# vocdoni/gnark-crypto-primitives

Measured on AMD Instinct MI355X. Metric: proofs/sec, Arbo-160 Poseidon SMT-verifier circuit, Groth16/BN254, higher is better.
Workload: dtype u32x8 Montgomery (254-bit integer)

## Files before the change

gnark_crypto_primitives_amd/csrc/api.hip:

```cpp
#include <algorithm>

#include "zkmi_internal.h"
#include "comb_plan.h"
#include "ff29.h"
#include "ec29.h"

using namespace zk;

namespace zk {

int ensure_scratch(zkmi_ctx* ctx, DevBuf& s, size_t bytes, void** out) {
  if (s.bytes < bytes) {
    if (s.p) {
      hipStreamSynchronize(ctx->stream);
      if (ctx->stream2) hipStreamSynchronize(ctx->stream2);
      if (ctx->stream3) hipStreamSynchronize(ctx->stream3);
      hipFree(s.p);
      s.p = nullptr;
      s.bytes = 0;
    }
    hipError_t e = hipMalloc(&s.p, bytes);
    if (e != hipSuccess) {
      ctx->err = "hipMalloc(" + std::to_string(bytes) + " B) failed: " + hipGetErrorString(e) +
                 " (the working set of this batch does not fit beside the MSM tables: load the key"
                 " with zkmi_pk_desc.max_batch >= the batch size, or with a table_budget_bytes cap)";
      s.p = nullptr;
      return ZKMI_ERR_OOM;
    }
    s.bytes = bytes;
  }
  if (out) *out = s.p;
  return ZKMI_OK;
}

int require_idle(zkmi_ctx* ctx) {
  if (!ctx->sets[0].pending && !ctx->sets[1].pending) return ZKMI_OK;
  ctx->err = "a submitted prove batch is in flight; collect it first";
  return ZKMI_ERR_ARG;
}

template <class P>
__global__ __launch_bounds__(256) void field_mul_kernel(const Fp<P>* a, const Fp<P>* b, Fp<P>* r,
                                                        size_t n) {
  size_t i = (size_t)blockIdx.x * blockDim.x + threadIdx.x;
  const size_t stride = (size_t)gridDim.x * blockDim.x;
  for (; i < n; i += stride) r[i] = mul(a[i], b[i]);
}

template <class P>
// ... 207 lines not shown
  const size_t Bp = round_up(batch, 64);
  const SetBytes sb = prove_set_bytes(value_rows, (size_t)1 << pk->log_n, n_staged, batch, Bp);
  int rc;
  for (zkmi_ctx::ProveSet* T : {&ctx->sets[ctx->next_submit ^ 1], &S}) {
    if (T->pending) continue;
    if ((rc = ensure_scratch(ctx, T->slots, sb.slots)) || (rc = ensure_scratch(ctx, T->a, sb.abc)) ||
        (rc = ensure_scratch(ctx, T->b, sb.abc)) || (rc = ensure_scratch(ctx, T->c, sb.abc)) ||
        (rc = ensure_scratch(ctx, T->misc, sb.misc)) ||
        (rc = ensure_scratch(ctx, T->sums, sums_bytes(Bp))))
      return rc;
  }
  char* const staged = (char*)S.misc.p + Bp * 100;
  S.rs = S.misc.p;
  S.st = (char*)S.misc.p + Bp * 96;
  if (stage) *stage = staged;
  S.heavy_enqueued = false;
  S.batch = batch;
  S.Bp = Bp;
  S.pk = pk;
  *main = ctx->stream;
  ctx->stream = ctx->stream2;
  hipEventRecord(S.ev0, ctx->stream);
  const void* rs_dev;
  rc = device_view(ctx, rs, batch * 64, staged + batch * n_staged * 32, &rs_dev);
  if (!rc) rc = transpose_in(ctx, rs_dev, S.rs, 2, batch, Bp, 32);
  return rc ? prove_set_end(ctx, *main, rc) : ZKMI_OK;
}

int prove_set_end(zkmi_ctx* ctx, hipStream_t main, int rc) {
  zkmi_ctx::ProveSet& S = ctx->sets[ctx->next_submit];
  hipEventRecord(S.ev1, ctx->stream);
  ctx->stream = main;
  if (rc) {
    hipStreamSynchronize(ctx->stream2);
    return rc;
  }
  S.pending = true;
  ctx->next_submit ^= 1;
  return ZKMI_OK;
}

}

extern "C" {

int zkmi_init(int device, zkmi_ctx** out) {
  if (!out) return ZKMI_ERR_ARG;
  *out = nullptr;
  int count = 0;
  if (hipGetDeviceCount(&count) != hipSuccess || count <= 0) return ZKMI_ERR_NO_DEVICE;
  if (device < 0 || device >= count) return ZKMI_ERR_ARG;
  if (hipSetDevice(device) != hipSuccess) return ZKMI_ERR_HIP;
  auto* ctx = new zkmi_ctx();
  ctx->device = device;
  if (hipStreamCreateWithFlags(&ctx->stream, hipStreamNonBlocking) != hipSuccess) {
    delete ctx;
    return ZKMI_ERR_HIP;
  }
  if (hipStreamCreateWithFlags(&ctx->stream2, hipStreamNonBlocking) != hipSuccess) {
    hipStreamDestroy(ctx->stream);
    delete ctx;
    return ZKMI_ERR_HIP;
  }
  if (hipStreamCreateWithFlags(&ctx->stream3, hipStreamNonBlocking) != hipSuccess) {
    hipStreamDestroy(ctx->stream2);
    hipStreamDestroy(ctx->stream);
    delete ctx;
    return ZKMI_ERR_HIP;
  }
  for (auto& st : ctx->sets) {
    hipEventCreate(&st.ev0);
    hipEventCreate(&st.ev1);
    for (auto& e : st.evq) hipEventCreate(&e);
    for (auto& e : st.eva) hipEventCreate(&e);
    for (auto& p : st.msm_ev) {
      hipEventCreate(&p[0]);
      hipEventCreate(&p[1]);
    }
  }
  for (auto& e : ctx->ev) hipEventCreate(&e);
  for (auto& e : ctx->part_ev) hipEventCreateWithFlags(&e, hipEventDisableTiming);
  for (auto& e : ctx->acc_ev) hipEventCreateWithFlags(&e, hipEventDisableTiming);
  ctx->plans.reserve(32);
  *out = ctx;
  return ZKMI_OK;
}

void zkmi_destroy(zkmi_ctx* ctx) {
  if (!ctx) return;
  hipSetDevice(ctx->device);
  hipStreamSynchronize(ctx->stream);
  hipStreamSynchronize(ctx->stream2);
  hipStreamSynchronize(ctx->stream3);
  for (auto& st : ctx->sets) {
    if (st.ev0) hipEventDestroy(st.ev0);
    if (st.ev1) hipEventDestroy(st.ev1);
    for (auto& e : st.evq)
      if (e) hipEventDestroy(e);
    for (auto& e : st.eva)
      if (e) hipEventDestroy(e);
    for (auto& p : st.msm_ev) {
      if (p[0]) hipEventDestroy(p[0]);
      if (p[1]) hipEventDestroy(p[1]);
    }
  }
  hipStreamDestroy(ctx->stream2);
  hipStreamDestroy(ctx->stream3);
  for (auto& p : ctx->plans) free_plan(p);
  for (auto& st : ctx->sets)
    for (DevBuf* b : {&st.slots, &st.a, &st.b, &st.c, &st.misc, &st.sums, &st.commit})
      if (b->p) hipFree(b->p);
  for (DevBuf* b : {&ctx->ntt_tmp, &ctx->build_tmp, &ctx->msm_digits, &ctx->msm_sint,
                    &ctx->msm_rowvar, &ctx->msm_part[0], &ctx->msm_part[1], &ctx->side_part2, &ctx->side_part3})
    if (b->p) hipFree(b->p);
  witness_ring_free(ctx);
  for (auto& e : ctx->ev)
    if (e) hipEventDestroy(e);
  for (auto& e : ctx->part_ev)
    if (e) hipEventDestroy(e);
  for (auto& e : ctx->acc_ev)
    if (e) hipEventDestroy(e);
  hipStreamDestroy(ctx->stream);
  delete ctx;
}

const char* zkmi_last_error(zkmi_ctx* ctx) { return ctx ? ctx->err.c_str() : "null context"; }

int zkmi_sync(zkmi_ctx* ctx) {
  ZK_HIP(hipStreamSynchronize(ctx->stream));
  return ZKMI_OK;
}

void* zkmi_stream(zkmi_ctx* ctx) { return (void*)ctx->stream; }

int zkmi_field_mul(zkmi_ctx* ctx, int which, const void* a, const void* b, void* r, size_t n) {
  ZK_HIP(hipSetDevice(ctx->device));
  Staged sa(ctx), sb(ctx), sr(ctx);
  int rc;
  if ((rc = sa.in(a, n * 32)) || (rc = sb.in(b, n * 32)) || (rc = sr.out(r, n * 32))) return rc;
  if (n == 0) return ZKMI_OK;
  unsigned g = (unsigned)((n + 255) / 256);
  if (g > 8192) g = 8192;
  if (which == 0)
    hipLaunchKernelGGL((field_mul_kernel<FrParams>), dim3(g), dim3(256), 0, ctx->stream,
                       (const Fr*)sa.dev, (const Fr*)sb.dev, (Fr*)sr.dev, n);
  else
    hipLaunchKernelGGL((field_mul_kernel<FqParams>), dim3(g), dim3(256), 0, ctx->stream,
                       (const Fq*)sa.dev, (const Fq*)sb.dev, (Fq*)sr.dev, n);
  ZK_HIP(hipGetLastError());
  if ((rc = sr.finish())) return rc;
  ZK_HIP(hipStreamSynchronize(ctx->stream));
  return ZKMI_OK;
}
// ... 137 lines not shown
    if (rc != ZKMI_ERR_OOM || !may_relax) return rc;
    if (plan.comb) {
      if (plan.comb <= 8) return rc;
      plan = plan_comb(plan.comb - 1, plan.comb_signed != 0);
    } else if (plan.shared) {
      if (plan.bits[0] <= 4) return rc;
      plan = plan_shared(plan.bits[0] - 1);
    } else {
      if (plan.W >= 64) return rc;
      plan = plan_with_windows(plan.W + 1);
    }
  }
}

static bool window_bits_ok(int wb) {
  return wb == 0 || (wb >= 2 && wb <= 16) || (wb >= 104 && wb <= 116) ||
         (wb >= 202 && wb <= 220) || (wb >= 303 && wb <= 321);
}
static WinPlan plan_explicit(int wb) {
  return wb >= 300   ? plan_comb(wb - 300, true)
         : wb >= 200 ? plan_comb(wb - 200, false)
         : wb >= 100 ? plan_shared(wb - 100)
                     : plan_uniform(wb);
}
static double prove_working_set_bytes(uint32_t log_n, size_t n_slots, size_t n_in, size_t max_batch,
                                      size_t n_msm_max, size_t n_commitments) {
  const size_t Bp = round_up(max_batch ? max_batch : 1024, 64);
  const size_t n = (size_t)1 << log_n;
  const SetBytes sb = prove_set_bytes(n_slots, n, n_in, Bp, Bp);
  const double set = (double)(sb.slots + 3 * sb.abc + sb.misc + sums_bytes(Bp) +
                              commit_buffer_bytes(n_commitments, Bp));
  const double digits = 254.0 * (double)((n_msm_max + 15) / 16) * Bp * 4;
  const double sint = (double)n_msm_max * Bp * 32;
  const double partials = 2 * 21.0 * 254 * Bp * 256;
  const double ring = 3.0 * std::max(68e6, (double)n_in * 32 * 64);
  return 2 * set + (double)n * Bp * 32 + digits + sint + partials + ring + 2e9 + 1e9;
}
static double free_hbm_bytes() {
  size_t free_b = 0, total_b = 0;
  if (hipMemGetInfo(&free_b, &total_b) != hipSuccess) free_b = (size_t)64 << 30;
  return (double)free_b;
}
static double usable_table_bytes_standalone(size_t n) {
  const double ws = (double)n * 1024 * 32 * 2 + 254.0 * ((n + 15) / 16) * 1024 * 4 +
                    21.0 * 254 * 1024 * 256 + 3e9;
  const double usable = free_hbm_bytes() - ws;
  return usable > 0 ? usable : 0.0;
}

int zkmi_msm_bases_load(zkmi_ctx* ctx, int group, const void* bases, size_t n, int window_bits,
                        zkmi_msm_bases** out) {
  return zkmi_msm_bases_load_image(ctx, group, bases, n, window_bits, 0, out);
}

int zkmi_msm_bases_load_image(zkmi_ctx* ctx, int group, const void* bases, size_t n,
                              int window_bits, int image, zkmi_msm_bases** out) {
  ZK_HIP(hipSetDevice(ctx->device));
  if (!out) return ZKMI_ERR_ARG;
  if (image != 0 && image != 1) {
    ctx->err = "image must be 0 (x * 2^256) or 1 (x * 2^261)";
    return ZKMI_ERR_ARG;
  }
  if (!window_bits_ok(window_bits)) {
    ctx->err = "window_bits must be 0 (auto), in [2,16], 100 + [4,16], 200 + [2,20] or 300 + [3,21]";
    return ZKMI_ERR_ARG;
  }
  Staged sb(ctx);
// ... 596 lines not shown
    }
    if (!rc) rc = solve_rows(ctx, cs, slots, a, b, c, st, Bp, begin, cs->n_rows);
    if (!rc) rc = commit_finish_submit(ctx, S);
  }
  return prove_set_end(ctx, main, rc);
}

static int enqueue_heavy(zkmi_ctx* ctx, int si) {
  zkmi_ctx::ProveSet& S = ctx->sets[si];
  const zkmi_pk* pk = S.pk;
  const bool fd = S.f_domain;
  const size_t Bp = S.Bp, batch = S.batch, n = (size_t)1 << pk->log_n;
  NttPlan* plan;
  int rc = get_plan(ctx, (int)pk->log_n, &plan);
  if (rc) return rc;
  void* t0;
  if ((rc = ensure_scratch(ctx, ctx->ntt_tmp, n * Bp * 32, &t0))) return rc;
  SumsView v(S.sums.p, Bp);
  Fr* rs_bi = (Fr*)S.rs;
  Fr* slots = (Fr*)S.slots.p;
  ZK_HIP(hipStreamWaitEvent(ctx->stream, S.ev1, 0));
  hipEventRecord(S.evq[0], ctx->stream);
  Fr* h;
  if ((rc = pk->folded ? compute_ab_coset_bi(ctx, plan, (Fr*)S.a.p, (Fr*)S.b.p, (Fr*)t0, Bp,
                                             S.n_constraints, &h, fd)
                       : compute_h_bi(ctx, plan, (Fr*)S.a.p, (Fr*)S.b.p, (Fr*)S.c.p, (Fr*)t0, Bp,
                                      S.n_constraints, &h, fd)))
    return rc;
  hipEventRecord(S.evq[1], ctx->stream);
  S.msm_ev_used = 0;
  ctx->msm_ev_set = si;
  const bool d1 = pk->Z->plan.shared || pk->Z->plan.comb;
  const bool d2 = pk->B2->plan.shared || pk->B2->plan.comb;
  hipStream_t q3 = ctx->stream3;
  uint8_t* rv = nullptr;
  if (pk->A->plan.comb || pk->B2->plan.comb) {
    void* p;
    if ((rc = ensure_scratch(ctx, ctx->msm_rowvar, pk->n_wires, &p)) ||
        (rc = msm_rows_vary(ctx, slots, pk->n_wires, Bp, batch, (uint8_t*)p))) {
      ctx->msm_ev_set = -1;
      return rc;
    }
    rv = (uint8_t*)p;
  }
  if ((rc = msm_run(ctx, pk->A, slots, pk->a_wire, Bp, batch, v.sA, fd, d1 ? v.w1[0] : nullptr, q3,
                    rv)) ||
      (rc = msm_run(ctx, pk->B1, slots, pk->b_wire, Bp, batch, v.sB1, fd, d1 ? v.w1[1] : nullptr, q3,
                    rv)) ||
      (rc = msm_run(ctx, pk->K, slots, pk->k_wire, Bp, batch, v.sK, fd, d1 ? v.w1[2] : nullptr, q3,
                    rv)) ||
      (rc = msm_run(ctx, pk->Z, h, nullptr, Bp, batch, v.sZ, false, d1 ? v.w1[3] : nullptr, q3,
                    nullptr, true))) {
    ctx->msm_ev_set = -1;
    return rc;
  }
  hipEventRecord(S.evq[2], ctx->stream);
  rc = msm_run(ctx, pk->B2, slots, pk->b_wire, Bp, batch, v.sB2, fd, d2 ? v.w2 : nullptr, q3, rv);
  ctx->msm_ev_set = -1;
  if (rc) return rc;
  hipEventRecord(S.evq[3], ctx->stream);
  {
    hipStream_t main_stream = ctx->stream;
    ZK_HIP(hipStreamWaitEvent(q3, S.ev1, 0));
    ctx->stream = q3;
    hipLaunchKernelGGL(rs_prep_kernel, dim3((unsigned)(Bp / 64)), dim3(64), 0, q3, rs_bi, Bp);
    (void)((rc = msm_run(ctx, pk->D1, rs_bi, pk->idx3 + 0, Bp, batch, v.tR)) ||
           (rc = msm_run(ctx, pk->D1, rs_bi, pk->idx3 + 1, Bp, batch, v.tS)) ||
           (rc = msm_run(ctx, pk->D1, rs_bi, pk->idx3 + 2, Bp, batch, v.tNRS)) ||
           (rc = msm_run(ctx, pk->D2, rs_bi, pk->idx3 + 1, Bp, batch, v.tS2)));
    ctx->stream = main_stream;
    if (rc) return rc;
  }
  if ((rc = commit_pok(ctx, S))) return rc;
  hipEventRecord(S.evq[4], ctx->stream);
  S.heavy_enqueued = true;
  return ZKMI_OK;
}

int zkmi_prove_collect(zkmi_ctx* ctx, void* proofs_out, int32_t* status_out) {
  return zkmi_prove_collect_ex(ctx, proofs_out, status_out, nullptr);
}

int zkmi_prove_collect_ex(zkmi_ctx* ctx, void* proofs_out, int32_t* status_out,
                          void* commitments_out) {
  ZK_HIP(hipSetDevice(ctx->device));
  const int si = ctx->next_collect;
  zkmi_ctx::ProveSet& S = ctx->sets[si];
  if (!S.pending) {
    ctx->err = "prove: nothing submitted";
    return ZKMI_ERR_ARG;
  }
  if (!S.pk->commits.empty() && !commitments_out) {
    ctx->err = "prove: this key has commitments: collect with zkmi_prove_collect_ex";
    return ZKMI_ERR_ARG;
  }
  const zkmi_pk* pk = S.pk;
  const size_t batch = S.batch, Bp = S.Bp;
  int rc;
  if (!S.heavy_enqueued && (rc = enqueue_heavy(ctx, si))) return rc;
  SumsView v(S.sums.p, Bp);
  hipStream_t q3 = ctx->stream3;
  ZK_HIP(hipStreamWaitEvent(q3, S.evq[4], 0));
  hipEventRecord(S.eva[0], q3);
  if (pk->Z->plan.shared || pk->Z->plan.comb) {
    void* ws[4] = {v.w1[0], v.w1[1], v.w1[2], v.w1[3]};
    void* os[4] = {v.sA, v.sB1, v.sK, v.sZ};
    const zkmi_msm_bases* ms[4] = {pk->A, pk->B1, pk->K, pk->Z};
    bool same = true;
    for (int i = 0; i < 3; i++)
      same = same && (ms[i]->plan.comb != 0) == (pk->Z->plan.comb != 0) &&
             ms[i]->plan.comb_signed == pk->Z->plan.comb_signed &&
             (pk->Z->plan.comb || (ms[i]->plan.shared && ms[i]->plan.bits[0] == pk->Z->plan.bits[0]));
    if (same) {
      if ((rc = msm_horner_run(ctx, q3, 4, ms, ws, os, Bp))) return rc;
    } else {
      for (int i = 0; i < 4; i++)
        if ((rc = msm_horner_run(ctx, q3, 1, ms + i, ws + i, os + i, Bp))) return rc;
    }
  }
  if (pk->B2->plan.shared || pk->B2->plan.comb) {
    void* ws[1] = {v.w2};
    void* os[1] = {v.sB2};
    const zkmi_msm_bases* ms[1] = {pk->B2};
    if ((rc = msm_horner_run(ctx, q3, 1, ms, ws, os, Bp))) return rc;
  }
  PkConsts pc{pk->alpha, pk->beta1, pk->beta2};
  hipLaunchKernelGGL(assemble_kernel, dim3((unsigned)(Bp / 64)), dim3(64), 0, q3, v.sA, v.sB1, v.sK,
                     v.sZ, v.tR, v.tS, v.tNRS, (const Fr*)S.rs, Bp, pc, v.proofs);
  hipLaunchKernelGGL(assemble_g2_kernel, dim3((unsigned)(Bp / 64)), dim3(64), 0, q3, v.sB2, v.tS2,
                     Bp, pk->beta2, v.proofs);
  ZK_HIP(hipGetLastError());
  ZK_HIP(hipMemcpyAsync(proofs_out, v.proofs, batch * 256, hipMemcpyDefault, q3));
  ZK_HIP(hipMemcpyAsync(status_out, S.st, batch * 4, hipMemcpyDefault, q3));
  if (const size_t nc = pk->commits.size()) {
    const size_t pitch = (nc + 1) * 64;
// ... 47 lines not shown
```

gnark_crypto_primitives_amd/csrc/msm_impl.h:

```cpp
#pragma once
#include "zkmi_internal.h"
#include "ec29.h"
#include "comb_sign.h"

namespace zk {

ZK_HD Fq to_r261_domain(const Fq& x) {
  Fq k;
#pragma unroll
  for (int i = 0; i < 8; i++) k.v[i] = Fq29Params::k261(i);
  return mul(x, k);
}
ZK_HD Fq2 to_r261_domain(const Fq2& x) { return Fq2{to_r261_domain(x.c0), to_r261_domain(x.c1)}; }

template <class F>
struct SegInv {
  F *szz, *szzz, *spre;
  size_t T;
  F pref = F::one();
  __device__ SegInv(F* scratch, uint32_t t, uint32_t T_, uint32_t seg_len)
      : szz(scratch + t), szzz(scratch + (size_t)seg_len * T_ + t),
        spre(scratch + (size_t)2 * seg_len * T_ + t), T(T_) {}
  __device__ void push(Affine<F>* seg, uint32_t d, const F& x, const F& y, const F& zz,
                       const F& zzz) {
    seg[d].x = x;
    seg[d].y = y;
    szz[d * T] = zz;
    szzz[d * T] = zzz;
    spre[d * T] = pref;
    pref = mul(pref, zzz);
  }
  __device__ void finish(Affine<F>* seg, uint32_t len) {
    F inv = inverse(pref);
    for (uint32_t d = len; d-- > 0;) {
      const F zzz = szzz[d * T];
      const F izzz = mul(inv, spre[d * T]);
// ... 827 lines not shown
  size_t chunks = want;
  if (chunks < 1) chunks = 1;
  if (chunks > items) chunks = items;
  const uint32_t per_chunk = (uint32_t)((items + chunks - 1) / chunks);
  chunks = (items + per_chunk - 1) / per_chunk;
  uint32_t group = 1;
  while ((size_t)group * group < chunks) group++;
  return {chunks, per_chunk, group, (uint32_t)((chunks + group - 1) / group)};
}

template <class F>
static void reduce_partials(hipStream_t stream, const XYZZ<F>* partial, XYZZ<F>* mid, XYZZ<F>* out,
                            size_t Bp, const ChunkSplit& cs, int W, const XYZZ<F>* addend,
                            const uint32_t* counts) {
  const Part29<F>* in = (const Part29<F>*)partial;
  uint32_t count = (uint32_t)cs.chunks, div = 1;
  if (cs.ngroups > 1) {
    hipLaunchKernelGGL((msm_reduce<F, false>), dim3((unsigned)(Bp / 64), cs.ngroups, (unsigned)W),
                       dim3(64), 0, stream, in, Bp, count, cs.group, (Part29<F>*)mid,
                       (size_t)count * Bp, (size_t)cs.ngroups * Bp, (const Part29<F>*)nullptr, counts,
                       (uint32_t)cs.chunks, div);
    in = (const Part29<F>*)mid;
    count = cs.ngroups;
    div = cs.group;
  }
  hipLaunchKernelGGL((msm_reduce<F, true>), dim3((unsigned)(Bp / 64), 1, (unsigned)W), dim3(64), 0,
                     stream, in, Bp, count, count, out, (size_t)count * Bp, Bp,
                     (const Part29<F>*)addend, counts, (uint32_t)cs.chunks, div);
}

template <class F>
struct PartView {
  XYZZ<F> *partial, *mid, *wsum, *usum;
  uint32_t* counts;
  static size_t bytes(const ChunkSplit& cs, int W, size_t Bp, bool common_sums) {
    return ((cs.chunks + cs.ngroups + 1) * W * Bp + (common_sums ? W : 0)) * sizeof(XYZZ<F>) +
           (common_sums ? 2 * sizeof(uint32_t) : 0);
  }
  PartView(void* base, const ChunkSplit& cs, int W, size_t Bp) {
    partial = (XYZZ<F>*)base;
    mid = partial + cs.chunks * W * Bp;
    wsum = mid + (size_t)cs.ngroups * W * Bp;
    usum = wsum + (size_t)W * Bp;
    counts = (uint32_t*)(usum + W);
  }
};

static inline int wait_partials_free(zkmi_ctx* ctx, int pb) {
  if (ctx->part_ev_valid[pb]) {
    ZK_HIP(hipStreamWaitEvent(ctx->stream, ctx->part_ev[pb], 0));
    ctx->part_ev_valid[pb] = false;
  }
  return ZKMI_OK;
}

static inline hipEvent_t acc_timer_begin(zkmi_ctx* ctx, const zkmi_msm_bases* bases) {
  if (ctx->msm_ev_set < 0) return nullptr;
  zkmi_ctx::ProveSet& es = ctx->sets[ctx->msm_ev_set];
  if (es.msm_ev_used >= 8) return nullptr;
  const int ev = es.msm_ev_used++;
  es.msm_ev_group[ev] = bases->group;
  hipEventRecord(es.msm_ev[ev][0], ctx->stream);
  return es.msm_ev[ev][1];
}
static inline void acc_timer_end(zkmi_ctx* ctx, hipEvent_t end) {
  if (end) hipEventRecord(end, ctx->stream);
}

template <class F>
int run_comb(zkmi_ctx* ctx, const zkmi_msm_bases* bases, const Fr* scalars, const uint32_t* row_idx,
             size_t Bp, size_t batch, XYZZ<F>* out, bool scalars_f, XYZZ<F>* wsum_out,
             hipStream_t finish_stream, const uint8_t* row_varies, bool dense) {
  const size_t n = bases->n;
  const uint32_t k = bases->plan.comb;
  const bool sg = bases->plan.comb_signed != 0;
  const size_t G = bases->n_groups;
  const int W = bases->plan.W;
  const size_t comb_factor = bases->chunk_factor ? bases->chunk_factor : 16;
  const ChunkSplit cs = split_chunks(G, comb_factor * 262144 / Bp / (size_t)W);
  void *part, *digits, *sint;
  const bool defer = wsum_out && finish_stream && finish_stream != ctx->stream;
  const int pb = defer ? (int)(ctx->part_next++ & 1u) : 0;
  int rc = ensure_scratch(ctx, ctx->msm_part[pb], PartView<F>::bytes(cs, W, Bp, true), &part);
  if (rc) return rc;
  if ((rc = wait_partials_free(ctx, pb))) return rc;
  if ((rc = ensure_scratch(ctx, ctx->msm_digits,
                           ((size_t)W * G * Bp + (size_t)(W + 3) * G) * sizeof(uint32_t) + n,
                           &digits)))
    return rc;
  uint32_t* d0 = (uint32_t*)digits + (size_t)W * G * Bp;
  uint32_t* vlist = d0 + (size_t)W * G;
  uint32_t* ulist = vlist + G;
  uint32_t* vpos = ulist + G;
  const PartView<F> pv(part, cs, W, Bp);
  uint32_t* counts = pv.counts;
  XYZZ<F>* wsum = wsum_out ? wsum_out : pv.wsum;
  const unsigned bx = (Bp % 256 == 0) ? 256 : 64;
  const dim3 dgrid((unsigned)(Bp / bx), (unsigned)(G < 8192 ? G : 8192));
  const uint8_t* flags = row_varies;
  const uint32_t* flag_idx = row_idx;
  if (!flags && !dense) {
    uint8_t* own = (uint8_t*)(vpos + G);
    hipLaunchKernelGGL(rows_vary_kernel, dim3((unsigned)((n + 3) / 4)), dim3(256), 0, ctx->stream,
                       scalars, row_idx, (uint32_t)n, Bp, batch, own);
    flags = own;
    flag_idx = nullptr;
  }
  hipLaunchKernelGGL(comb_split_kernel, dim3(1), dim3(1024), 0, ctx->stream, flags, flag_idx,
                     (uint32_t)n, k, dense ? 1 : 0, (uint32_t)G, vlist, ulist, vpos, counts);
  const Fr* dsrc = scalars;
  const uint32_t* didx = row_idx;
  if (!(sg && scalars_f == (bases->image == MSM_IMAGE_F))) {
    if ((rc = ensure_scratch(ctx, ctx->msm_sint, n * Bp * sizeof(Fr), &sint))) return rc;
    Fr29 kk = Fr29::zero();
    if (!sg)
      kk.v[0] = scalars_f ? 1 : 32;
    else
      for (int i = 0; i < 9; i++) kk.v[i] = scalars_f ? Fr29Params::c256(i) : Fr29Params::c266(i);
    const dim3 sgrid((unsigned)(Bp / bx), (unsigned)(n < 16384 ? n : 16384));
    hipLaunchKernelGGL(comb_scalars_kernel, sgrid, dim3(bx), 0, ctx->stream, scalars, row_idx, Bp,
                       (uint32_t)n, kk, (const uint8_t*)bases->inf, (Fr*)sint);
    dsrc = (const Fr*)sint;
    didx = nullptr;
  }
  hipLaunchKernelGGL((sg ? comb_digits_kernel<21, true> : comb_digits_kernel<20, false>), dgrid,
                     dim3(bx), 0, ctx->stream, dsrc, didx, Bp, (uint32_t)n, k, (uint32_t)G,
                     (const uint32_t*)vpos, (uint32_t*)digits, d0);
  const hipEvent_t timed = acc_timer_begin(ctx, bases);
  const dim3 grid((unsigned)(Bp / bx), (unsigned)W, (unsigned)cs.chunks);
  const uint32_t per_group = 1u << (sg ? k - 1 : k);
  const bool ci = bases->entries_may_be_inf != 0;
  const auto sums = ci ? (sg ? comb_common_sums<F, true, true> : comb_common_sums<F, true, false>)
                       : (sg ? comb_common_sums<F, false, true> : comb_common_sums<F, false, false>);
  const auto accumulate =
      ci ? (sg ? msm_accumulate_comb<F, true, true> : msm_accumulate_comb<F, true, false>)
         : (sg ? msm_accumulate_comb<F, false, true> : msm_accumulate_comb<F, false, false>);
  hipLaunchKernelGGL(sums, dim3((unsigned)W), dim3(256), 0, ctx->stream,
                     (const Affine<F>*)bases->table, (const uint32_t*)d0, (uint32_t)G,
                     (const uint32_t*)ulist, (const uint32_t*)counts, per_group,
                     (Part29<F>*)pv.usum);
  hipLaunchKernelGGL(accumulate, grid, dim3(bx), 0, ctx->stream, (const Affine<F>*)bases->table,
                     (const uint32_t*)digits, Bp, (uint32_t)G, (const uint32_t*)vlist,
                     (const uint32_t*)counts, per_group, (Part29<F>*)pv.partial);
  acc_timer_end(ctx, timed);
  hipStream_t rq = ctx->stream;
  if (defer) {
    ZK_HIP(hipEventRecord(ctx->acc_ev[pb], ctx->stream));
    ZK_HIP(hipStreamWaitEvent(finish_stream, ctx->acc_ev[pb], 0));
    rq = finish_stream;
  }
  reduce_partials<F>(rq, pv.partial, pv.mid, wsum, Bp, cs, W, pv.usum, counts);
  if (defer) {
    ZK_HIP(hipEventRecord(ctx->part_ev[pb], finish_stream));
    ctx->part_ev_valid[pb] = true;
  }
  if (!wsum_out) {
    HornerArgsRW<F> ha{};
    ha.wsum[0] = wsum;
    ha.out[0] = out;
    ha.stotal[0] = stotal_of(bases, F{});
    launch_comb_horner<F>(ctx->stream, ha, 1, Bp, bases->plan);
  }
  ZK_HIP(hipGetLastError());
  return ZKMI_OK;
}

template <class F>
int run_shared(zkmi_ctx* ctx, const zkmi_msm_bases* bases, const Fr* scalars,
               const uint32_t* row_idx, size_t Bp, XYZZ<F>* out, bool scalars_f,
               XYZZ<F>* wsum_out) {
  const size_t n = bases->n;
  const WinPlan& plan = bases->plan;
  const int W = plan.W;
  Fr koff = Fr::zero();
  {
    uint32_t pos = 0;
    for (int j = 0; j < W; j++) {
      const uint32_t bit = pos + plan.bits[j] - 1;
      koff.v[bit >> 5] |= 1u << (bit & 31);
      pos += plan.bits[j];
    }
  }
  const size_t shared_factor = bases->chunk_factor ? bases->chunk_factor : 8;
  const ChunkSplit cs = split_chunks(n, shared_factor * 262144 / Bp / (size_t)W);
  void *part, *digits;
  int rc = ensure_scratch(ctx, ctx->msm_part[0], PartView<F>::bytes(cs, W, Bp, false), &part);
  if (rc) return rc;
  if ((rc = wait_partials_free(ctx, 0))) return rc;
  if ((rc = ensure_scratch(ctx, ctx->msm_digits, (size_t)W * n * Bp * sizeof(int16_t), &digits)))
    return rc;
  const PartView<F> pv(part, cs, W, Bp);
  XYZZ<F>* wsum = wsum_out ? wsum_out : pv.wsum;
  const unsigned bx = (Bp % 256 == 0) ? 256 : 64;
  hipLaunchKernelGGL(msm_digits_kernel,
                     dim3((unsigned)(Bp / bx), (unsigned)(n < 16384 ? n : 16384)), dim3(bx), 0,
                     ctx->stream, scalars, row_idx, Bp, (uint32_t)n, plan,
                     (int32_t)(scalars_f ? 1 : 32), koff, (const uint8_t*)bases->inf,
                     (int16_t*)digits);
  const hipEvent_t timed = acc_timer_begin(ctx, bases);
  hipLaunchKernelGGL((msm_accumulate_shared<F>),
                     dim3((unsigned)(Bp / bx), (unsigned)W, (unsigned)cs.chunks), dim3(bx), 0,
                     ctx->stream, (const Affine<F>*)bases->table, (const int16_t*)digits, Bp,
                     (uint32_t)n, cs.per_chunk, plan.per_base, (Part29<F>*)pv.partial);
  acc_timer_end(ctx, timed);
  reduce_partials<F>(ctx->stream, pv.partial, pv.mid, wsum, Bp, cs, W, nullptr, nullptr);
  if (!wsum_out) {
    HornerArgs<F> ha{};
    ha.wsum[0] = wsum;
    ha.out[0] = out;
    hipLaunchKernelGGL((msm_horner<F>), dim3((unsigned)(Bp / 64), 1), dim3(64), 0, ctx->stream,
                       ha, Bp, plan);
  }
  ZK_HIP(hipGetLastError());
  return ZKMI_OK;
}

template <class F>
int run_windows(zkmi_ctx* ctx, const zkmi_msm_bases* bases, const Fr* scalars,
                const uint32_t* row_idx, size_t Bp, XYZZ<F>* out, bool scalars_f) {
  const size_t n = bases->n;
  Fr kmul = Fr::zero();
  kmul.v[0] = 1;
  if (scalars_f) {
    Fr t = Fr::zero();
// ... 43 lines not shown
```

gnark_crypto_primitives_amd/csrc/r1cs_solve.hip:

```cpp
#include <algorithm>
#include <new>
#include <string>
#include <vector>

#include "zkmi_internal.h"
#include "ff29.h"
#include "ff29_asm.h"
#include "r1cs_plan.h"

using namespace zk;

struct zkmi_r1cs_solver {
  uint32_t n_wires = 0, n_constraints = 0, n_inputs = 0, n_instr = 0, S = 1;
  uint32_t n_records = 0;
  bool ext = false;
  bool emul = false;
  std::vector<R1csCommit> commits;
  uint32_t longest = 0, n_inversions = 0;
  uint64_t n_terms = 0;
  uint4* records = nullptr;
  uint2* terms = nullptr;
  Fr* coeffs = nullptr;
  uint32_t* outs = nullptr;
};
// ... 323 lines not shown
  s->n_constraints = m->n_constraints;
  s->n_inputs = d->n_public - 1 + d->n_secret;
  s->n_instr = plan.n_instr;
  s->n_records = (uint32_t)plan.records.size() - 1;
  s->ext = plan.ext;
  s->emul = plan.emul;
  s->commits = std::move(plan.commits);
  s->S = plan.S;
  s->longest = plan.longest;
  s->n_inversions = plan.n_inversions;
  s->n_terms = plan.n_terms;
  static_assert(sizeof(R1csRecord) == 2 * sizeof(uint4), "record = two quads");
  if (!upload(&s->records, plan.records.data(), plan.records.size() * 2) ||
      !upload(&s->terms, plan.terms.data(), plan.terms.size()) ||
      !upload(&s->coeffs, plan.coeffs.data(), plan.coeffs.size()) ||
      !upload(&s->outs, plan.outs.data(), plan.outs.size())) {
    ctx->err = "r1cs solver: device upload failed";
    zkmi_r1cs_solver_free(ctx, s);
    return ZKMI_ERR_HIP;
  }
  *out = s;
  return ZKMI_OK;
}

}

extern "C" {

void zkmi_r1cs_solver_free(zkmi_ctx* ctx, zkmi_r1cs_solver* s) {
  if (!s) return;
  if (ctx) {
    hipSetDevice(ctx->device);
    hipStreamSynchronize(ctx->stream);
    if (ctx->stream2) hipStreamSynchronize(ctx->stream2);
  }
  if (s->records) hipFree(s->records);
  if (s->terms) hipFree(s->terms);
  if (s->coeffs) hipFree(s->coeffs);
  if (s->outs) hipFree(s->outs);
  delete s;
}

int zkmi_r1cs_solver_load(zkmi_ctx* ctx, const zkmi_r1cs* r1cs, const zkmi_r1cs_solver_desc* desc,
                          zkmi_r1cs_solver** out) {
  ZK_HIP(hipSetDevice(ctx->device));
  if (!r1cs || !desc || !out) {
    ctx->err = "r1cs solver: null argument";
    return ZKMI_ERR_ARG;
  }
  *out = nullptr;
  try {
    return solver_load(ctx, r1cs, desc, out);
  } catch (const std::bad_alloc&) {
    ctx->err = "r1cs solver: out of host memory while building the plan";
    return ZKMI_ERR_OOM;
  }
}

int zkmi_r1cs_solver_info(const zkmi_r1cs_solver* s, uint64_t* info) {
  if (!s || !info) return ZKMI_ERR_ARG;
  info[0] = s->n_instr;
  info[1] = s->S;
  info[2] = s->n_terms;
  info[3] = s->longest;
  info[4] = s->n_inversions;
  info[5] = s->n_wires;
  info[6] = s->n_constraints;
// ... 119 lines not shown
```

gnark_crypto_primitives_amd/csrc/witness.hip:

```cpp
#include <algorithm>
#include <cstring>
#include <thread>

#include "zkmi_internal.h"
#include "ff29.h"
#if defined(__HIP_DEVICE_COMPILE__)
#include "ff29_asm.h"
#endif

using namespace zk;

namespace zk {

int pointer_kind(const void* p) {
  hipPointerAttribute_t attr;
  hipError_t e = hipPointerGetAttributes(&attr, p);
  if (e != hipSuccess) {
    (void)hipGetLastError();
    return PTR_PAGEABLE;
  }
  if (attr.type == hipMemoryTypeDevice || attr.type == hipMemoryTypeManaged) return PTR_DEVICE;
  if (attr.type == hipMemoryTypeHost) return PTR_PINNED;
  return PTR_PAGEABLE;
}
// ... 173 lines not shown
}

extern "C" {

void* zkmi_host_alloc(zkmi_ctx* ctx, size_t bytes) {
  if (!ctx || bytes == 0) return nullptr;
  if (hipSetDevice(ctx->device) != hipSuccess) return nullptr;
  void* p = nullptr;
  if (hipHostMalloc(&p, bytes, hipHostMallocDefault) != hipSuccess) {
    (void)hipGetLastError();
    ctx->err = "zkmi_host_alloc: hipHostMalloc(" + std::to_string(bytes) + " B) failed";
    return nullptr;
  }
  return p;
}

void zkmi_host_free(zkmi_ctx* ctx, void* p) {
  if (!p) return;
  if (ctx) hipSetDevice(ctx->device);
  hipHostFree(p);
}

int zkmi_set_copy_threads(zkmi_ctx* ctx, int threads) {
  if (!ctx || threads < 0 || threads > 64) return ZKMI_ERR_ARG;
  ctx->copy_threads = threads;
  return ZKMI_OK;
}

void zkmi_r1cs_free(zkmi_ctx* ctx, zkmi_r1cs* m) {
  if (!m) return;
  if (ctx) {
    hipSetDevice(ctx->device);
    hipStreamSynchronize(ctx->stream);
    if (ctx->stream2) hipStreamSynchronize(ctx->stream2);
  }
  for (int s = 0; s < 3; s++) {
    if (m->ptr[s]) hipFree(m->ptr[s]);
    if (m->terms[s]) hipFree(m->terms[s]);
  }
  if (m->coeffs) hipFree(m->coeffs);
  delete m;
}

int zkmi_r1cs_load(zkmi_ctx* ctx, const zkmi_r1cs_desc* d, zkmi_r1cs** out) {
  ZK_HIP(hipSetDevice(ctx->device));
  if (!d || !out) return ZKMI_ERR_ARG;
  *out = nullptr;
  if (d->n_constraints == 0 || d->n_wires == 0 || d->n_coeffs == 0 || d->n_coeffs >= (1u << 30) ||
      !d->coeffs) {
    ctx->err = "r1cs: n_constraints, n_wires and n_coeffs (< 2^30) must be positive";
    return ZKMI_ERR_ARG;
  }
  std::vector<Fr> coeffs(d->n_coeffs);
  if (hipMemcpy(coeffs.data(), d->coeffs, (size_t)d->n_coeffs * 32, hipMemcpyDefault) != hipSuccess) {
    ctx->err = "r1cs: cannot read the coefficient table";
    return ZKMI_ERR_HIP;
  }
  const Fr one = Fr::one(), minus_one = neg(Fr::one());
  std::vector<uint8_t> kind(d->n_coeffs);
  for (uint32_t i = 0; i < d->n_coeffs; i++) {
    const Fr& x = coeffs[i];
    bool lt = false;
    for (int j = 7; j >= 0; j--) {
      if (x.v[j] != FrParams::p(j)) {
        lt = x.v[j] < FrParams::p(j);
        break;
      }
// ... 157 lines not shown
```

gnark_crypto_primitives_amd/csrc/zkmi_internal.h:

```cpp
#pragma once
#include <hip/hip_runtime.h>
#include <stdint.h>
#include <string>
#include <utility>
#include <vector>

#include "../../include/zkmi.h"
#include "ec.h"
#include "vprog.h"

namespace zk {


struct DevBuf {
  void* p = nullptr;
  size_t bytes = 0;
};

struct NttPlan {
  int log_n = 0;
  Fr* tw_fwd = nullptr;
  Fr* tw_inv = nullptr;
  Fr* coset_fwd = nullptr;
  Fr* coset_inv = nullptr;
  Fr* coset_inv_den = nullptr;
  Fr n_inv;
  Fr den;
  Fr ninv_den;
  Fr* tw29_fwd = nullptr;
  Fr* tw29_inv = nullptr;
  Fr* coset29_fwd = nullptr;
  Fr* coset29n_fwd = nullptr;
};

}

struct zkmi_ctx {
  int device = 0;
  hipStream_t stream = nullptr;
  std::string err;
  std::vector<zk::NttPlan> plans;
  hipEvent_t ev[8] = {};
  double timings[8] = {};
  zk::DevBuf ntt_tmp;
  zk::DevBuf build_tmp;
  zk::DevBuf msm_digits, msm_sint;
  zk::DevBuf msm_rowvar;
  zk::DevBuf msm_part[2];
  zk::DevBuf side_part2;
  zk::DevBuf side_part3;
  hipStream_t stream2 = nullptr, stream3 = nullptr;
  struct ProveSet {
    bool pending = false;
    bool heavy_enqueued = false;
    zk::DevBuf slots, a, b, c, misc, sums, commit;
    hipEvent_t evq[5] = {};
    hipEvent_t eva[2] = {};
    hipEvent_t msm_ev[8][2] = {};
    int msm_ev_group[8] = {};
    int msm_ev_used = 0;
    size_t batch = 0, Bp = 0;
    const zkmi_pk* pk = nullptr;
    const zkmi_cs* cs = nullptr;
    size_t n_constraints = 0;
    bool f_domain = true;
    void *rs = nullptr, *st = nullptr;
    hipEvent_t ev0 = nullptr, ev1 = nullptr;
    void *commit_pts = nullptr, *commit_ch = nullptr, *commit_pok = nullptr, *commit_acc = nullptr;
    std::vector<zk::Fr> commit_host;
  } sets[2];
  int next_submit = 0, next_collect = 0;
  int msm_ev_set = -1;
  hipEvent_t part_ev[2] = {}, acc_ev[2] = {};
  bool part_ev_valid[2] = {false, false};
  unsigned part_next = 0;
  struct StageRing {
    void* pinned[3] = {};
    void* dev[3] = {};
    hipEvent_t done[3] = {};
    bool busy[3] = {false, false, false};
    size_t bytes = 0;
    unsigned next = 0;
  } ring;
  int copy_threads = 0;
};

struct WinPlan {
  int W = 0;
  uint32_t per_base = 0;
  uint8_t bits[64] = {};
  uint32_t off[64] = {};
  uint8_t shared = 0;
  uint8_t comb = 0;
  uint8_t comb_signed = 0;
};

struct zkmi_msm_bases {
  int group = 1;
  size_t n = 0;
  WinPlan plan;
  void* table = nullptr;
  size_t table_bytes = 0;
  uint8_t* inf = nullptr;
  size_t n_groups = 0;
  int entries_may_be_inf = 0;
  uint32_t chunk_factor = 0;
// ... 48 lines not shown
__device__ __forceinline__ Fr bi_ld(const Fr* base, size_t row, size_t b, size_t Bp) {
  const uint4* p = reinterpret_cast<const uint4*>(base) + row * 2 * Bp + b;
  const uint4 lo = p[0], hi = p[Bp];
  Fr r;
  r.v[0] = lo.x; r.v[1] = lo.y; r.v[2] = lo.z; r.v[3] = lo.w;
  r.v[4] = hi.x; r.v[5] = hi.y; r.v[6] = hi.z; r.v[7] = hi.w;
  return r;
}
__device__ __forceinline__ void bi_st(Fr* base, size_t row, size_t b, size_t Bp, const Fr& x) {
  uint4* p = reinterpret_cast<uint4*>(base) + row * 2 * Bp + b;
  p[0] = make_uint4(x.v[0], x.v[1], x.v[2], x.v[3]);
  p[Bp] = make_uint4(x.v[4], x.v[5], x.v[6], x.v[7]);
}
__device__ __forceinline__ void bi_st_nt(Fr* base, size_t row, size_t b, size_t Bp, const Fr& x) {
  typedef uint32_t u32x4 __attribute__((ext_vector_type(4)));
  u32x4* p = reinterpret_cast<u32x4*>(base) + row * 2 * Bp + b;
  u32x4 lo = {x.v[0], x.v[1], x.v[2], x.v[3]}, hi = {x.v[4], x.v[5], x.v[6], x.v[7]};
  __builtin_nontemporal_store(lo, p);
  __builtin_nontemporal_store(hi, p + Bp);
}
#endif

#define ZK_HIP(call)                                                         \
  do {                                                                       \
    hipError_t _e = (call);                                                  \
    if (_e != hipSuccess) {                                                  \
      ctx->err = std::string(#call) + ": " + hipGetErrorString(_e);          \
      return ZKMI_ERR_HIP;                                                   \
    }                                                                        \
  } while (0)

static inline size_t round_up(size_t x, size_t m) { return (x + m - 1) / m * m; }

int ensure_scratch(zkmi_ctx* ctx, DevBuf& buf, size_t bytes, void** out = nullptr);
int require_idle(zkmi_ctx* ctx);
enum { PTR_PAGEABLE = 0, PTR_PINNED = 1, PTR_DEVICE = 2 };
int pointer_kind(const void* p);
void witness_ring_free(zkmi_ctx* ctx);

struct Staged {
  zkmi_ctx* ctx;
  void* dev = nullptr;
  void* host = nullptr;
  size_t bytes = 0;
  bool owned = false;
  Staged(zkmi_ctx* c) : ctx(c) {}
  int in(const void* p, size_t n) {
    bytes = n;
    if (n == 0) return ZKMI_OK;
    if (pointer_kind(p) == PTR_DEVICE) {
      dev = const_cast<void*>(p);
      return ZKMI_OK;
    }
    ZK_HIP(hipMalloc(&dev, n));
    owned = true;
    ZK_HIP(hipMemcpyAsync(dev, p, n, hipMemcpyHostToDevice, ctx->stream));
    return ZKMI_OK;
  }
  int out(void* p, size_t n) {
    bytes = n;
    if (n == 0) return ZKMI_OK;
    if (pointer_kind(p) == PTR_DEVICE) {
      dev = p;
      return ZKMI_OK;
    }
    ZK_HIP(hipMalloc(&dev, n));
// ... 92 lines not shown
```

Measured before the change: 8860.

## Move comb MSM common-sum kernel and reductions onto a dedicated fourth stream

Adds a fourth stream that takes the deferred per-MSM finishing work (reductions) away from stream3. The comb path's common-sums kernel now also runs on that finishing stream, gated by a new digits-ready event, so it no longer sits ahead of the heavy accumulate kernel on the main stream. It is skipped entirely in the dense case. To make this safe, d0 and ulist move from the shared digits scratch into the double-buffered partials buffer. A tail event makes the later stream3 work wait for stream4. The aim is more overlap between MSM accumulation and its side work, at the cost of more streams, events and scratch memory.

```diff
diff --git a/gnark_crypto_primitives_amd/csrc/api.hip b/gnark_crypto_primitives_amd/csrc/api.hip
--- a/gnark_crypto_primitives_amd/csrc/api.hip
+++ b/gnark_crypto_primitives_amd/csrc/api.hip
@@ -9,12 +9,16 @@
 
 namespace zk {
 
+void sync_side_streams(zkmi_ctx* ctx) {
+  for (hipStream_t q : {ctx->stream2, ctx->stream3, ctx->stream4})
+    if (q) hipStreamSynchronize(q);
+}
+
 int ensure_scratch(zkmi_ctx* ctx, DevBuf& s, size_t bytes, void** out) {
   if (s.bytes < bytes) {
     if (s.p) {
       hipStreamSynchronize(ctx->stream);
-      if (ctx->stream2) hipStreamSynchronize(ctx->stream2);
-      if (ctx->stream3) hipStreamSynchronize(ctx->stream3);
+      sync_side_streams(ctx);
       hipFree(s.p);
       s.p = nullptr;
       s.bytes = 0;
@@ -288,7 +292,7 @@
   hipEventRecord(S.ev1, ctx->stream);
   ctx->stream = main;
   if (rc) {
-    hipStreamSynchronize(ctx->stream2);
+    sync_side_streams(ctx);
     return rc;
   }
   S.pending = true;
@@ -324,11 +328,19 @@
     delete ctx;
     return ZKMI_ERR_HIP;
   }
+  if (hipStreamCreateWithFlags(&ctx->stream4, hipStreamNonBlocking) != hipSuccess) {
+    hipStreamDestroy(ctx->stream3);
+    hipStreamDestroy(ctx->stream2);
+    hipStreamDestroy(ctx->stream);
+    delete ctx;
+    return ZKMI_ERR_HIP;
+  }
   for (auto& st : ctx->sets) {
     hipEventCreate(&st.ev0);
     hipEventCreate(&st.ev1);
     for (auto& e : st.evq) hipEventCreate(&e);
     for (auto& e : st.eva) hipEventCreate(&e);
+    hipEventCreateWithFlags(&st.tail_ev, hipEventDisableTiming);
     for (auto& p : st.msm_ev) {
       hipEventCreate(&p[0]);
       hipEventCreate(&p[1]);
@@ -337,6 +349,7 @@
   for (auto& e : ctx->ev) hipEventCreate(&e);
   for (auto& e : ctx->part_ev) hipEventCreateWithFlags(&e, hipEventDisableTiming);
   for (auto& e : ctx->acc_ev) hipEventCreateWithFlags(&e, hipEventDisableTiming);
+  for (auto& e : ctx->dig_ev) hipEventCreateWithFlags(&e, hipEventDisableTiming);
   ctx->plans.reserve(32);
   *out = ctx;
   return ZKMI_OK;
@@ -346,8 +359,7 @@
   if (!ctx) return;
   hipSetDevice(ctx->device);
   hipStreamSynchronize(ctx->stream);
-  hipStreamSynchronize(ctx->stream2);
-  hipStreamSynchronize(ctx->stream3);
+  sync_side_streams(ctx);
   for (auto& st : ctx->sets) {
     if (st.ev0) hipEventDestroy(st.ev0);
     if (st.ev1) hipEventDestroy(st.ev1);
@@ -355,6 +367,7 @@
       if (e) hipEventDestroy(e);
     for (auto& e : st.eva)
       if (e) hipEventDestroy(e);
+    if (st.tail_ev) hipEventDestroy(st.tail_ev);
     for (auto& p : st.msm_ev) {
       if (p[0]) hipEventDestroy(p[0]);
       if (p[1]) hipEventDestroy(p[1]);
@@ -362,6 +375,7 @@
   }
   hipStreamDestroy(ctx->stream2);
   hipStreamDestroy(ctx->stream3);
+  hipStreamDestroy(ctx->stream4);
   for (auto& p : ctx->plans) free_plan(p);
   for (auto& st : ctx->sets)
     for (DevBuf* b : {&st.slots, &st.a, &st.b, &st.c, &st.misc, &st.sums, &st.commit})
@@ -375,6 +389,8 @@
   for (auto& e : ctx->part_ev)
     if (e) hipEventDestroy(e);
   for (auto& e : ctx->acc_ev)
+    if (e) hipEventDestroy(e);
+  for (auto& e : ctx->dig_ev)
     if (e) hipEventDestroy(e);
   hipStreamDestroy(ctx->stream);
   delete ctx;
@@ -578,7 +594,7 @@
                               commit_buffer_bytes(n_commitments, Bp));
   const double digits = 254.0 * (double)((n_msm_max + 15) / 16) * Bp * 4;
   const double sint = (double)n_msm_max * Bp * 32;
-  const double partials = 2 * 21.0 * 254 * Bp * 256;
+  const double partials = 2 * (21.0 * 254 * Bp * 256 + 256.0 * (double)((n_msm_max + 15) / 16) * 4);
   const double ring = 3.0 * std::max(68e6, (double)n_in * 32 * 64);
   return 2 * set + (double)n * Bp * 32 + digits + sint + partials + ring + 2e9 + 1e9;
 }
@@ -1241,7 +1257,7 @@
   ctx->msm_ev_set = si;
   const bool d1 = pk->Z->plan.shared || pk->Z->plan.comb;
   const bool d2 = pk->B2->plan.shared || pk->B2->plan.comb;
-  hipStream_t q3 = ctx->stream3;
+  hipStream_t q3 = ctx->stream3, q4 = ctx->stream4;
   uint8_t* rv = nullptr;
   if (pk->A->plan.comb || pk->B2->plan.comb) {
     void* p;
@@ -1252,22 +1268,23 @@
     }
     rv = (uint8_t*)p;
   }
-  if ((rc = msm_run(ctx, pk->A, slots, pk->a_wire, Bp, batch, v.sA, fd, d1 ? v.w1[0] : nullptr, q3,
+  if ((rc = msm_run(ctx, pk->A, slots, pk->a_wire, Bp, batch, v.sA, fd, d1 ? v.w1[0] : nullptr, q4,
                     rv)) ||
-      (rc = msm_run(ctx, pk->B1, slots, pk->b_wire, Bp, batch, v.sB1, fd, d1 ? v.w1[1] : nullptr, q3,
+      (rc = msm_run(ctx, pk->B1, slots, pk->b_wire, Bp, batch, v.sB1, fd, d1 ? v.w1[1] : nullptr, q4,
                     rv)) ||
-      (rc = msm_run(ctx, pk->K, slots, pk->k_wire, Bp, batch, v.sK, fd, d1 ? v.w1[2] : nullptr, q3,
+      (rc = msm_run(ctx, pk->K, slots, pk->k_wire, Bp, batch, v.sK, fd, d1 ? v.w1[2] : nullptr, q4,
                     rv)) ||
-      (rc = msm_run(ctx, pk->Z, h, nullptr, Bp, batch, v.sZ, false, d1 ? v.w1[3] : nullptr, q3,
+      (rc = msm_run(ctx, pk->Z, h, nullptr, Bp, batch, v.sZ, false, d1 ? v.w1[3] : nullptr, q4,
                     nullptr, true))) {
     ctx->msm_ev_set = -1;
     return rc;
   }
   hipEventRecord(S.evq[2], ctx->stream);
-  rc = msm_run(ctx, pk->B2, slots, pk->b_wire, Bp, batch, v.sB2, fd, d2 ? v.w2 : nullptr, q3, rv);
+  rc = msm_run(ctx, pk->B2, slots, pk->b_wire, Bp, batch, v.sB2, fd, d2 ? v.w2 : nullptr, q4, rv);
   ctx->msm_ev_set = -1;
   if (rc) return rc;
   hipEventRecord(S.evq[3], ctx->stream);
+  ZK_HIP(hipEventRecord(S.tail_ev, q4));
   {
     hipStream_t main_stream = ctx->stream;
     ZK_HIP(hipStreamWaitEvent(q3, S.ev1, 0));
@@ -1310,6 +1327,7 @@
   SumsView v(S.sums.p, Bp);
   hipStream_t q3 = ctx->stream3;
   ZK_HIP(hipStreamWaitEvent(q3, S.evq[4], 0));
+  ZK_HIP(hipStreamWaitEvent(q3, S.tail_ev, 0));
   hipEventRecord(S.eva[0], q3);
   if (pk->Z->plan.shared || pk->Z->plan.comb) {
     void* ws[4] = {v.w1[0], v.w1[1], v.w1[2], v.w1[3]};
diff --git a/gnark_crypto_primitives_amd/csrc/msm_impl.h b/gnark_crypto_primitives_amd/csrc/msm_impl.h
--- a/gnark_crypto_primitives_amd/csrc/msm_impl.h
+++ b/gnark_crypto_primitives_amd/csrc/msm_impl.h
@@ -2,6 +2,7 @@
 #include "zkmi_internal.h"
 #include "ec29.h"
 #include "comb_sign.h"
+#include "msm_part_layout.h"
 
 namespace zk {
 
@@ -895,17 +896,24 @@
 template <class F>
 struct PartView {
   XYZZ<F> *partial, *mid, *wsum, *usum;
-  uint32_t* counts;
-  static size_t bytes(const ChunkSplit& cs, int W, size_t Bp, bool common_sums) {
-    return ((cs.chunks + cs.ngroups + 1) * W * Bp + (common_sums ? W : 0)) * sizeof(XYZZ<F>) +
-           (common_sums ? 2 * sizeof(uint32_t) : 0);
-  }
-  PartView(void* base, const ChunkSplit& cs, int W, size_t Bp) {
-    partial = (XYZZ<F>*)base;
-    mid = partial + cs.chunks * W * Bp;
-    wsum = mid + (size_t)cs.ngroups * W * Bp;
-    usum = wsum + (size_t)W * Bp;
-    counts = (uint32_t*)(usum + W);
+  uint32_t *counts, *d0, *ulist;
+  static MsmPartLayout layout(const ChunkSplit& cs, int W, size_t Bp, size_t G, bool common_sums) {
+    return msm_part_layout(sizeof(XYZZ<F>), cs.chunks, cs.ngroups, (size_t)W, Bp, G, common_sums);
+  }
+  static size_t bytes(const ChunkSplit& cs, int W, size_t Bp, size_t G, bool common_sums) {
+    return layout(cs, W, Bp, G, common_sums).bytes();
+  }
+  PartView(void* base, const ChunkSplit& cs, int W, size_t Bp, size_t G, bool common_sums) {
+    static_assert(sizeof(XYZZ<F>) == sizeof(Part29<F>), "packed accumulators share the regions");
+    const MsmPartLayout l = layout(cs, W, Bp, G, common_sums);
+    char* m = (char*)base;
+    partial = (XYZZ<F>*)(m + l.off[MSM_PART_PARTIAL]);
+    mid = (XYZZ<F>*)(m + l.off[MSM_PART_MID]);
+    wsum = (XYZZ<F>*)(m + l.off[MSM_PART_WSUM]);
+    usum = (XYZZ<F>*)(m + l.off[MSM_PART_USUM]);
+    counts = (uint32_t*)(m + l.off[MSM_PART_COUNTS]);
+    d0 = (uint32_t*)(m + l.off[MSM_PART_D0]);
+    ulist = (uint32_t*)(m + l.off[MSM_PART_ULIST]);
   }
 };
 
@@ -944,19 +952,16 @@
   void *part, *digits, *sint;
   const bool defer = wsum_out && finish_stream && finish_stream != ctx->stream;
   const int pb = defer ? (int)(ctx->part_next++ & 1u) : 0;
-  int rc = ensure_scratch(ctx, ctx->msm_part[pb], PartView<F>::bytes(cs, W, Bp, true), &part);
+  int rc = ensure_scratch(ctx, ctx->msm_part[pb], PartView<F>::bytes(cs, W, Bp, G, true), &part);
   if (rc) return rc;
   if ((rc = wait_partials_free(ctx, pb))) return rc;
   if ((rc = ensure_scratch(ctx, ctx->msm_digits,
-                           ((size_t)W * G * Bp + (size_t)(W + 3) * G) * sizeof(uint32_t) + n,
-                           &digits)))
+                           ((size_t)W * G * Bp + (size_t)2 * G) * sizeof(uint32_t) + n, &digits)))
     return rc;
-  uint32_t* d0 = (uint32_t*)digits + (size_t)W * G * Bp;
-  uint32_t* vlist = d0 + (size_t)W * G;
-  uint32_t* ulist = vlist + G;
-  uint32_t* vpos = ulist + G;
-  const PartView<F> pv(part, cs, W, Bp);
-  uint32_t* counts = pv.counts;
+  uint32_t* vlist = (uint32_t*)digits + (size_t)W * G * Bp;
+  uint32_t* vpos = vlist + G;
+  const PartView<F> pv(part, cs, W, Bp, G, true);
+  uint32_t *counts = pv.counts, *d0 = pv.d0, *ulist = pv.ulist;
   XYZZ<F>* wsum = wsum_out ? wsum_out : pv.wsum;
   const unsigned bx = (Bp % 256 == 0) ? 256 : 64;
   const dim3 dgrid((unsigned)(Bp / bx), (unsigned)(G < 8192 ? G : 8192));
@@ -989,7 +994,6 @@
   hipLaunchKernelGGL((sg ? comb_digits_kernel<21, true> : comb_digits_kernel<20, false>), dgrid,
                      dim3(bx), 0, ctx->stream, dsrc, didx, Bp, (uint32_t)n, k, (uint32_t)G,
                      (const uint32_t*)vpos, (uint32_t*)digits, d0);
-  const hipEvent_t timed = acc_timer_begin(ctx, bases);
   const dim3 grid((unsigned)(Bp / bx), (unsigned)W, (unsigned)cs.chunks);
   const uint32_t per_group = 1u << (sg ? k - 1 : k);
   const bool ci = bases->entries_may_be_inf != 0;
@@ -998,21 +1002,28 @@
   const auto accumulate =
       ci ? (sg ? msm_accumulate_comb<F, true, true> : msm_accumulate_comb<F, true, false>)
          : (sg ? msm_accumulate_comb<F, false, true> : msm_accumulate_comb<F, false, false>);
-  hipLaunchKernelGGL(sums, dim3((unsigned)W), dim3(256), 0, ctx->stream,
-                     (const Affine<F>*)bases->table, (const uint32_t*)d0, (uint32_t)G,
-                     (const uint32_t*)ulist, (const uint32_t*)counts, per_group,
-                     (Part29<F>*)pv.usum);
+  hipStream_t rq = defer ? finish_stream : ctx->stream;
+  const XYZZ<F>* addend = nullptr;
+  if (!dense) {
+    if (defer) {
+      ZK_HIP(hipEventRecord(ctx->dig_ev[pb], ctx->stream));
+      ZK_HIP(hipStreamWaitEvent(rq, ctx->dig_ev[pb], 0));
+    }
+    hipLaunchKernelGGL(sums, dim3((unsigned)W), dim3(256), 0, rq, (const Affine<F>*)bases->table,
+                       (const uint32_t*)d0, (uint32_t)G, (const uint32_t*)ulist,
+                       (const uint32_t*)counts, per_group, (Part29<F>*)pv.usum);
+    addend = pv.usum;
+  }
+  const hipEvent_t timed = acc_timer_begin(ctx, bases);
   hipLaunchKernelGGL(accumulate, grid, dim3(bx), 0, ctx->stream, (const Affine<F>*)bases->table,
                      (const uint32_t*)digits, Bp, (uint32_t)G, (const uint32_t*)vlist,
                      (const uint32_t*)counts, per_group, (Part29<F>*)pv.partial);
   acc_timer_end(ctx, timed);
-  hipStream_t rq = ctx->stream;
   if (defer) {
     ZK_HIP(hipEventRecord(ctx->acc_ev[pb], ctx->stream));
-    ZK_HIP(hipStreamWaitEvent(finish_stream, ctx->acc_ev[pb], 0));
-    rq = finish_stream;
-  }
-  reduce_partials<F>(rq, pv.partial, pv.mid, wsum, Bp, cs, W, pv.usum, counts);
+    ZK_HIP(hipStreamWaitEvent(rq, ctx->acc_ev[pb], 0));
+  }
+  reduce_partials<F>(rq, pv.partial, pv.mid, wsum, Bp, cs, W, addend, counts);
   if (defer) {
     ZK_HIP(hipEventRecord(ctx->part_ev[pb], finish_stream));
     ctx->part_ev_valid[pb] = true;
@@ -1047,12 +1058,12 @@
   const size_t shared_factor = bases->chunk_factor ? bases->chunk_factor : 8;
   const ChunkSplit cs = split_chunks(n, shared_factor * 262144 / Bp / (size_t)W);
   void *part, *digits;
-  int rc = ensure_scratch(ctx, ctx->msm_part[0], PartView<F>::bytes(cs, W, Bp, false), &part);
+  int rc = ensure_scratch(ctx, ctx->msm_part[0], PartView<F>::bytes(cs, W, Bp, 0, false), &part);
   if (rc) return rc;
   if ((rc = wait_partials_free(ctx, 0))) return rc;
   if ((rc = ensure_scratch(ctx, ctx->msm_digits, (size_t)W * n * Bp * sizeof(int16_t), &digits)))
     return rc;
-  const PartView<F> pv(part, cs, W, Bp);
+  const PartView<F> pv(part, cs, W, Bp, 0, false);
   XYZZ<F>* wsum = wsum_out ? wsum_out : pv.wsum;
   const unsigned bx = (Bp % 256 == 0) ? 256 : 64;
   hipLaunchKernelGGL(msm_digits_kernel,
diff --git a/gnark_crypto_primitives_amd/csrc/msm_part_layout.h b/gnark_crypto_primitives_amd/csrc/msm_part_layout.h
--- /dev/null
+++ b/gnark_crypto_primitives_amd/csrc/msm_part_layout.h
@@ -0,0 +1,52 @@
+#pragma once
+#include <cstddef>
+#include <cstdint>
+
+namespace zk {
+
+enum {
+  MSM_PART_PARTIAL = 0,
+  MSM_PART_MID,
+  MSM_PART_WSUM,
+  MSM_PART_USUM,
+  MSM_PART_COUNTS,
+  MSM_PART_D0,
+  MSM_PART_ULIST,
+  MSM_PART_REGIONS
+};
+
+struct MsmPartLayout {
+  size_t off[MSM_PART_REGIONS];
+  size_t size[MSM_PART_REGIONS];
+  size_t align[MSM_PART_REGIONS];
+  size_t bytes() const { return off[MSM_PART_REGIONS - 1] + size[MSM_PART_REGIONS - 1]; }
+};
+
+inline const char* msm_part_region_name(int r) {
+  static const char* const names[MSM_PART_REGIONS] = {"partial", "mid",  "wsum", "usum",
+                                                      "counts",  "d0",   "ulist"};
+  return names[r];
+}
+
+inline MsmPartLayout msm_part_layout(size_t elem, size_t chunks, size_t ngroups, size_t W, size_t Bp,
+                                     size_t G, bool common_sums) {
+  MsmPartLayout l;
+  const size_t u32 = sizeof(uint32_t);
+  const size_t size[MSM_PART_REGIONS] = {chunks * W * Bp * elem,
+                                         ngroups * W * Bp * elem,
+                                         W * Bp * elem,
+                                         common_sums ? W * elem : 0,
+                                         common_sums ? 2 * u32 : 0,
+                                         common_sums ? W * G * u32 : 0,
+                                         common_sums ? G * u32 : 0};
+  size_t at = 0;
+  for (int r = 0; r < MSM_PART_REGIONS; r++) {
+    l.off[r] = at;
+    l.size[r] = size[r];
+    l.align[r] = r <= MSM_PART_USUM ? elem : u32;
+    at += size[r];
+  }
+  return l;
+}
+
+}
diff --git a/gnark_crypto_primitives_amd/csrc/r1cs_solve.hip b/gnark_crypto_primitives_amd/csrc/r1cs_solve.hip
--- a/gnark_crypto_primitives_amd/csrc/r1cs_solve.hip
+++ b/gnark_crypto_primitives_amd/csrc/r1cs_solve.hip
@@ -379,7 +379,7 @@
   if (ctx) {
     hipSetDevice(ctx->device);
     hipStreamSynchronize(ctx->stream);
-    if (ctx->stream2) hipStreamSynchronize(ctx->stream2);
+    sync_side_streams(ctx);
   }
   if (s->records) hipFree(s->records);
   if (s->terms) hipFree(s->terms);
diff --git a/gnark_crypto_primitives_amd/csrc/witness.hip b/gnark_crypto_primitives_amd/csrc/witness.hip
--- a/gnark_crypto_primitives_amd/csrc/witness.hip
+++ b/gnark_crypto_primitives_amd/csrc/witness.hip
@@ -229,7 +229,7 @@
   if (ctx) {
     hipSetDevice(ctx->device);
     hipStreamSynchronize(ctx->stream);
-    if (ctx->stream2) hipStreamSynchronize(ctx->stream2);
+    sync_side_streams(ctx);
   }
   for (int s = 0; s < 3; s++) {
     if (m->ptr[s]) hipFree(m->ptr[s]);
diff --git a/gnark_crypto_primitives_amd/csrc/zkmi_internal.h b/gnark_crypto_primitives_amd/csrc/zkmi_internal.h
--- a/gnark_crypto_primitives_amd/csrc/zkmi_internal.h
+++ b/gnark_crypto_primitives_amd/csrc/zkmi_internal.h
@@ -49,13 +49,14 @@
   zk::DevBuf msm_part[2];
   zk::DevBuf side_part2;
   zk::DevBuf side_part3;
-  hipStream_t stream2 = nullptr, stream3 = nullptr;
+  hipStream_t stream2 = nullptr, stream3 = nullptr, stream4 = nullptr;
   struct ProveSet {
     bool pending = false;
     bool heavy_enqueued = false;
     zk::DevBuf slots, a, b, c, misc, sums, commit;
     hipEvent_t evq[5] = {};
     hipEvent_t eva[2] = {};
+    hipEvent_t tail_ev = nullptr;
     hipEvent_t msm_ev[8][2] = {};
     int msm_ev_group[8] = {};
     int msm_ev_used = 0;
@@ -71,7 +72,7 @@
   } sets[2];
   int next_submit = 0, next_collect = 0;
   int msm_ev_set = -1;
-  hipEvent_t part_ev[2] = {}, acc_ev[2] = {};
+  hipEvent_t part_ev[2] = {}, acc_ev[2] = {}, dig_ev[2] = {};
   bool part_ev_valid[2] = {false, false};
   unsigned part_next = 0;
   struct StageRing {
@@ -186,6 +187,7 @@
 
 static inline size_t round_up(size_t x, size_t m) { return (x + m - 1) / m * m; }
 
+void sync_side_streams(zkmi_ctx* ctx);
 int ensure_scratch(zkmi_ctx* ctx, DevBuf& buf, size_t bytes, void** out = nullptr);
 int require_idle(zkmi_ctx* ctx);
 enum { PTR_PAGEABLE = 0, PTR_PINNED = 1, PTR_DEVICE = 2 };
```

Measured after the change: 9134, median of 6. 3.1% higher.
